# NumericalEarth/Breeze.jl

Measured on AMD Instinct MI355X. Metric: grid-cells advanced/sec (tendency+Poisson step), 512^3 anelastic, higher is better.
Workload: dtype f64

## Files before the change

### breeze.jl_amd/csrc/bz_context.hip

```cpp
#include <cmath>
#include <cstdlib>
#include <cstring>

#include "bz_internal.h"

ProfileScope::ProfileScope(bz_ctx *c, const char *name) : ctx(c)
{
    if (!ctx->profiling || ctx->profile_mute) return;
    for (size_t s = 0; s < ctx->slots.size(); ++s)
        if (ctx->slots[s].name == name || std::strcmp(ctx->slots[s].name, name) == 0) slot = (int)s;
    if (slot < 0) {
        ctx->slots.emplace_back();
        ctx->slots.back().name = name;
        slot = (int)ctx->slots.size() - 1;
    }
    if (hipEventCreate(&e0) != hipSuccess || hipEventCreate(&e1) != hipSuccess) { slot = -1; return; }
    hipEventRecord(e0, ctx->stream);
}
ProfileScope::~ProfileScope()
{
    if (slot < 0) return;
    hipEventRecord(e1, ctx->stream);
    ctx->slots[slot].pending.emplace_back(e0, e1);
}
// ... 13 lines not shown
        }
        s.pending.clear();
    }
}

void bzi_read_tuning(bz_tuning &t)
{
    auto on = [](const char *n) { return getenv(n) != nullptr; };
    auto num = [](const char *n, int d) { const char *e = getenv(n); return e ? atoi(e) : d; };
    t.no_fused = on("BZ_NO_FUSED");
    t.no_fuse_rk = on("BZ_NO_FUSE_RK");
    t.no_lean = on("BZ_NO_LEAN");
    t.no_xcd = on("BZ_NO_XCD");
    t.no_k6_stored = on("BZ_NO_K6_STORED");
    t.no_closure_march = on("BZ_NO_CLOSURE_MARCH");
    t.no_dry_shortcut = on("BZ_NO_DRY_SHORTCUT");
    t.side_scalar = on("BZ_SIDE_SCALAR");
    t.no_fuse_forcing = on("BZ_NO_FUSE_FORCING");
    t.no_fold_forcing = on("BZ_NO_FOLD_FORCING");
    t.no_fuse_level_sums = on("BZ_NO_FUSE_LEVEL_SUMS");
    t.ac_xcd = num("BZ_AC_XCD", 1);
    t.ac_forward2 = num("BZ_AC_FWD2", 1);
    t.ac_pfold = num("BZ_AC_PFOLD", 1);
    t.ac_init_fold = num("BZ_AC_INIT_FOLD", 1);
    t.ac_pair_avg = num("BZ_AC_PAIR_AVG", 1);
    t.ac_rotate = num("BZ_AC_ROTATE", 1);
    t.ac_cfg = num("BZ_AC_CFG", 29);
    t.ac_bx = num("BZ_AC_BX", 128);
    t.no_tridiag_coop = on("BZ_NO_TRIDIAG_COOP");
    t.no_xfft = on("BZ_NO_XFFT");
    t.poisson_kxmajor = num("BZ_POISSON_KXMAJOR", 1);
    t.poisson_kx_pad = num("BZ_POISSON_KX_PAD", 1);
    t.poisson_kx_chunk_kb = num("BZ_POISSON_KX_CHUNK_KB", 0);
    t.poisson_chunk = num("BZ_POISSON_CHUNK", 0);
    t.no_generic_march = on("BZ_NO_GENERIC_MARCH");
    t.no_rho3d_exchange = on("BZ_NO_RHO3D_EXCHANGE");
    t.scalar_lds = num("BZ_SCALAR_LDS", 1);
    t.no_ac_fuse = on("BZ_NO_AC_FUSE");
    t.no_ac_end_fuse = on("BZ_NO_AC_END_FUSE");
    t.comm_no_overlap = on("BZ_COMM_NO_OVERLAP");
    t.comm_self_messages = on("BZ_COMM_SELF_MESSAGES");
    t.comm_no_side_scalar = on("BZ_COMM_NO_SIDE_SCALAR");
    t.nmc_store_always = on("BZ_NMC_STORE_ALWAYS");
    t.graph = num("BZ_GRAPH", -1);
    t.graph_debug = on("BZ_GRAPH_DEBUG");
}

extern "C" int bz_profile_enable(bz_ctx *ctx, int on)
{
    if (!ctx) return BZ_ERR_INVALID;
    if (!on) profile_drain(ctx);
    ctx->profiling = on != 0;
    return BZ_OK;
}
extern "C" int bz_profile_reset(bz_ctx *ctx)
{
    if (!ctx) return BZ_ERR_INVALID;
    profile_drain(ctx);
    for (auto &s : ctx->slots) { s.total_ms = 0.0; s.launches = 0; }
    return BZ_OK;
}
extern "C" int bz_profile_count(bz_ctx *ctx) { return ctx ? (int)ctx->slots.size() : 0; }
extern "C" int bz_profile_get(bz_ctx *ctx, int idx, const char **name, double *total_ms, int64_t *launches)
{
    if (!ctx || idx < 0 || idx >= (int)ctx->slots.size()) return BZ_ERR_INVALID;
    profile_drain(ctx);
// ... 331 lines not shown
```

### breeze.jl_amd/csrc/bz_fused.hip

```cpp
#include "bz_internal.h"

#define FX 64
#define FY 4

struct RKFieldsW {
    double *u[5];
    double *u0[5];
    const double *G[5];
};

template <bool FIRST>
__global__ __launch_bounds__(256) void k_rk3_rows(DevGrid g, RKFieldsW F, double dt, double alpha)
{
    const long long t = (long long)blockIdx.x * 256 + threadIdx.x;
    if (t >= (long long)g.Ny * g.Sx) return;
    const int k = blockIdx.y;
    const long long n = g.Sxy * (k + g.Hz) + (long long)g.Hy * g.Sx + t;
    const double oma = 1.0 - alpha;
#pragma unroll
    for (int f = 0; f < 5; ++f) {
        if (f == 2 && k == 0) continue;
        double u = F.u[f][n];
        if (FIRST) {
            F.u0[f][n] = u;
// ... 320 lines not shown
        if (!once[1]) { BZ_HIP(hipFuncSetAttribute((const void *)k_x_forward<0, 2>, hipFuncAttributeMaxDynamicSharedMemorySize, (int)lds)); once[1] = true; }
        if (rows) hipLaunchKernelGGL((k_x_forward<0, 2>), grid, block, lds, ctx->stream, g, rows, pu, pv, pw, dt, out, L, W, kc);
        else hipLaunchKernelGGL((k_x_forward<1, 2>), grid, block, lds, ctx->stream, g, rows, pu, pv, pw, dt, out, L, W, kc);
    } else if (rows) hipLaunchKernelGGL((k_x_forward<0, 1>), grid, block, lds, ctx->stream, g, rows, pu, pv, pw, dt, out, L, W, kc);
    else hipLaunchKernelGGL((k_x_forward<1, 1>), grid, block, lds, ctx->stream, g, rows, pu, pv, pw, dt, out, L, W, kc);
    BZ_LAUNCH_CHECK();
    return BZ_OK;
}

int bzi_xf_inverse(bz_ctx *ctx, const double *hat, double *phi, int blocks, int klo, int khi)
{
    const DevGrid &g = ctx->dg;
    if (khi <= 0) { klo = 0; khi = g.Nz; }
    const int n2 = g.Nx / 2, kc = xf_chunk(16, g);
    XfLayout L;
    L.nkx = blocks > 1 ? ctx->nkx : n2 + 1;
    L.nxp = blocks > 1 ? ctx->nkx * blocks : n2 + 1;
    L.blk = (long long)g.Nz * L.nkx * g.Ny;
    L.klo = klo; L.khi = khi;
    L.kxs = (ctx->kxmajor && blocks == 1 && !hat) ? (long long)(g.Nz + ctx->kx_pad) * g.Ny : 0;
    const double2 *in = (const double2 *)(hat ? hat : (const double *)ctx->d_hat);
    double *out = phi ? phi : ctx->d_rhs;
    const dim3 grid(g.Ny / XF_RB, (khi - klo + kc - 1) / kc), block(XF_RB * (n2 / 4));
    const size_t lds = xf_lds_bytes(n2);
    if (n2 / 4 > 64 || n2 % 3 == 0) {
        static bool once = false;
        if (!once) { BZ_HIP(hipFuncSetAttribute((const void *)k_x_inverse<2>, hipFuncAttributeMaxDynamicSharedMemorySize, (int)lds)); once = true; }
        hipLaunchKernelGGL(k_x_inverse<2>, grid, block, lds, ctx->stream, g, in, L, out, (const double2 *)ctx->d_wtab, kc);
    } else hipLaunchKernelGGL(k_x_inverse<1>, grid, block, lds, ctx->stream, g, in, L, out, (const double2 *)ctx->d_wtab, kc);
    BZ_LAUNCH_CHECK();
    return BZ_OK;
}

int bzi_rk3_fused(bz_ctx *ctx, const bz_state *s, const bz_prognostic *U0, const bz_prognostic *G, double dt,
                  double alpha, bool first)
{
    const DevGrid &g = ctx->dg;
    ProfileScope ps(ctx, first ? "ssp_rk3_substep+store_initial_state" : "ssp_rk3_substep");
    RKFieldsW F;
    F.u[0] = s->rho_u; F.u[1] = s->rho_v; F.u[2] = s->rho_w; F.u[3] = s->rho_theta; F.u[4] = s->rho_q;
    F.u0[0] = U0->rho_u; F.u0[1] = U0->rho_v; F.u0[2] = U0->rho_w; F.u0[3] = U0->rho_theta; F.u0[4] = U0->rho_q;
    F.G[0] = G->rho_u; F.G[1] = G->rho_v; F.G[2] = G->rho_w; F.G[3] = G->rho_theta; F.G[4] = G->rho_q;
    long long per_level = (long long)g.Ny * g.Sx;
    dim3 grid((unsigned)((per_level + 255) / 256), g.Nz), block(256);
    if (first)
        hipLaunchKernelGGL(k_rk3_rows<true>, grid, block, 0, ctx->stream, g, F, dt, alpha);
    else
        hipLaunchKernelGGL(k_rk3_rows<false>, grid, block, 0, ctx->stream, g, F, dt, alpha);
    BZ_LAUNCH_CHECK();
    return BZ_OK;
}

int bzi_poisson_source_fused(bz_ctx *ctx, const bz_state *s, double dt, double *rhs, const bz_prognostic *predictor)
{
    const DevGrid &g = ctx->dg;
    ProfileScope ps(ctx, "poisson_source_term");
    const int k0 = ctx->krn ? ctx->kr0 : 0, nk = ctx->krn ? ctx->krn : g.Nz;
    dim3 grid((g.Nx + 255) / 256, g.Ny, nk), block(256);
    hipLaunchKernelGGL(k_poisson_source_rows, grid, block, 0, ctx->stream, g, rhs ? rhs : ctx->d_rhs,
                       predictor ? predictor->rho_u : s->rho_u, predictor ? predictor->rho_v : s->rho_v,
                       predictor ? predictor->rho_w : s->rho_w, dt, k0);
    BZ_LAUNCH_CHECK();
    return BZ_OK;
}

int bzi_project_lean(bz_ctx *ctx, const bz_state *s, double dt, const double *phi_c, const double *phi_below,
// ... 58 lines not shown
```

### breeze.jl_amd/csrc/bz_internal.h

```cpp
#pragma once
#include <hip/hip_runtime.h>
#include <hipfft/hipfft.h>

#include <cstdint>
#include <cstdio>
#include <string>
#include <vector>

#include "../../include/breeze_hip.h"

struct ColPtr {
    const double *p = nullptr;
    ColPtr() = default;
    __host__ __device__ ColPtr(const double *q) : p(q) {}
    __host__ __device__ operator const double *() const { return p; }
#ifdef __HIPCC__
    typedef const double __attribute__((address_space(4))) *cptr;
    __device__ __forceinline__ double operator[](int k) const { return ((cptr)p)[k]; }
    __device__ __forceinline__ double operator[](long long k) const { return ((cptr)p)[k]; }
#endif
};

struct DevGrid {
    int Nx, Ny, Nz;
// ... 327 lines not shown

struct BzComm;
struct ProfileSlot {
    const char *name;
    double total_ms = 0.0;
    int64_t launches = 0;
    std::vector<std::pair<hipEvent_t, hipEvent_t>> pending;
};

struct bz_tuning {
    bool no_fused = false;
    bool no_fuse_rk = false;
    bool no_lean = false;
    bool no_xcd = false;
    bool no_closure_march = false;
    bool no_k6_stored = false;
    bool no_dry_shortcut = false;
    bool side_scalar = false;
    bool no_fuse_forcing = false;
    bool no_fold_forcing = false;
    int ac_xcd = 1;
    int ac_forward2 = 1;
    int ac_rotate = 1;
    int ac_pair_avg = 1;
    int ac_init_fold = 1;
    int ac_pfold = 1;
    int ac_bx = 128;
    int ac_cfg = 29;
    bool no_fuse_level_sums = false;
    bool no_tridiag_coop = false;
    bool no_xfft = false;
    int poisson_kxmajor = 1;
    int poisson_kx_chunk_kb = 0;
    int poisson_kx_pad = 1;
    int poisson_chunk = 0;
    int scalar_lds = 1;
    bool no_rho3d_exchange = false;
    bool no_generic_march = false;
    bool no_ac_fuse = false;
    bool no_ac_end_fuse = false;
    bool comm_no_overlap = false;
    bool comm_self_messages = false;
    bool comm_no_side_scalar = false;
    bool nmc_store_always = false;
    int graph = -1;
    bool graph_debug = false;
};
void bzi_read_tuning(bz_tuning &t);
#define BZ_REJECT_BOUNDED_Y(ctx, enabling, what)                                                                             \
    do {                                                                                                                     \
        if ((ctx) && (ctx)->dg.bounded_y && (enabling)) {                                                                                \
            (ctx)->last_error = what ": not implemented on a Bounded y (topology (Periodic, Bounded, Bounded))";            \
            return BZ_ERR_UNSUPPORTED;                                                                                       \
        }                                                                                                                    \
    } while (0)
#define BZ_REJECT_KINEMATIC(ctx, who)                                                                                        \
    do {                                                                                                                     \
        if ((ctx) && (ctx)->kinematic) {                                                                                     \
            (ctx)->last_error = who ": the context has PrescribedDynamics (no momentum, no pressure solve); use bz_time_steps_kinematic"; \
            return BZ_ERR_UNSUPPORTED;                                                                                       \
        }                                                                                                                    \
    } while (0)
#define BZ_HALO_XFACE 8
#define BZ_HALO_YFACE 4
struct bz_ctx;
bool bzi_lean_forcings_ok(const bz_ctx *ctx);

struct bz_ctx {
    bz_tuning tune;
    bz_grid grid;
    bz_constants constants;
    DevGrid dg;
    hipStream_t stream = nullptr;
    bool walls_lean_ok = false;
    int num_cus = 256;
    std::string last_error;

    double *d_columns = nullptr;
    int NXH = 0;
    hipfftHandle plan_fwd = 0, plan_inv = 0;
    hipfftDoubleComplex *d_dctx = nullptr;
    bool plans_ok = false;
    hipfftHandle plan_fwd_c = 0, plan_inv_c = 0;
    int pchunk = 0;
    int kr0 = 0, krn = 0;
    bool xf = false;
    bool xf_slab = false;
    void *d_wtab = nullptr;
    hipfftHandle plan_y = 0;
    bool kxmajor = false;
    int kx_cw = 0, kx_nch = 0, kx_pad = 0;
    hipfftHandle plan_yc = 0, plan_yc_last = 0;
    int profile_mute = 0;
    hipfftHandle slab_plan_x_fwd = 0, slab_plan_x_inv = 0, slab_plan_y = 0;
    bool slab_plans_ok = false;
    int slab_inv_ld = 0;
    double *d_rhs = nullptr;
    hipfftDoubleComplex *d_hat = nullptr;
    double *d_ibeta = nullptr;
    double *d_tfac = nullptr;
    double *d_lower = nullptr;
    double *d_scalar = nullptr;
    double *d_havg = nullptr;
    double *d_moments = nullptr;
    struct AzPlan *az = nullptr;
    int y_nranks = 1, y_rank = 0, nkx = 0, kx0 = 0, Ny_global = 0;
    bool slab_mode = false;
    bool tiled_tendencies = true;
    bool fuse_rk = true;
    bool G_is_predictor = false;
    bool fused_ok = true;
    int q_host = 0;
    int *h_qstate = nullptr;
    hipEvent_t ev_q = nullptr;
    bool q_pending = false;
    int *d_qstate = nullptr;
    bool diagnostics_stale = false;
    bool lean_step_last = false;
    bool lean = true;
    bool lean_xcd = true;
    hipStream_t side_stream = nullptr;
// ... 190 lines not shown
                       int32_t unpack, int sx, long long sxy);
int bzi_comm_join_pending(bz_ctx *ctx);
int bzi_refresh_diagnostics(bz_ctx *ctx, const bz_state *s, const char *who);
int bzi_kinematic_update_state(bz_ctx *ctx, const bz_state *s, const bz_prognostic *G, int compute_tendencies);
void bzi_kinematic_teardown(bz_ctx *ctx);
enum bz_tier { BZ_TIER_LEAN, BZ_TIER_FUSED_RK, BZ_TIER_FUSED, BZ_TIER_OPERATORS };
bz_tier bzi_anelastic_tier(const bz_ctx *ctx);
inline constexpr double BZ_SSP_RK3_ALPHA[3] = {1.0, 1.0 / 4.0, 2.0 / 3.0};
int bzi_zero_wall_faces(bz_ctx *ctx, const bz_prognostic *G, const bz_prognostic *U0 = nullptr);
int bzi_fused_rk_physics(bz_ctx *ctx, const bz_state *s, const bz_prognostic *G, double dt, double alpha, bool first, bool fold);
void bzi_lean_step_done(bz_ctx *ctx, bool diagnosed);
int bzi_scan_moisture(bz_ctx *ctx, const bz_state *s);
int bzi_scan_moisture_field(bz_ctx *ctx, const double *rho_q);
const int *bzi_moisture_state(const bz_ctx *ctx);
void bzi_moisture_unknown(bz_ctx *ctx);
struct LeanStage;
void bzi_lean_stage(const bz_state *s, const bz_prognostic *U0, const bz_prognostic *G, int stage, LeanStage *L);
int bzi_dist_time_step_compressible(bz_ctx *ctx, const bz_compressible_state *s, const bz_compressible_prognostic *U0,
                                    const bz_compressible_prognostic *G, const bz_acoustic_substepper *sub, double dt);
int bzi_compressible_store_initial_state(bz_ctx *ctx, const bz_compressible_state *s, const bz_compressible_prognostic *U0);
void bzi_comm_teardown(bz_ctx *ctx);
int bzi_comm_allreduce_sum(bz_ctx *ctx, double *buf, int n);
void bzi_lean_teardown(bz_ctx *ctx);
void bzi_poisson_teardown(bz_ctx *ctx);
int bzi_poisson_solve(bz_ctx *ctx, const bz_state *s, double dt);
int bzi_poisson_spectral(bz_ctx *ctx);
int bzi_poisson_from_momentum(bz_ctx *ctx, const bz_state *s, double dt, const bz_prognostic *predictor);
int bzi_fft_chunk(bz_ctx *ctx, int k0, bool forward);
int bzi_xf_forward(bz_ctx *ctx, const bz_state *s, double dt, const bz_prognostic *predictor, const double *rhs = nullptr,
                   double *hat = nullptr, int blocks = 1, int klo = 0, int khi = 0);
int bzi_xf_inverse(bz_ctx *ctx, const double *hat = nullptr, double *phi = nullptr, int blocks = 1, int klo = 0, int khi = 0);
int bzi_xf_y(bz_ctx *ctx, bool forward);
int bzi_tridiag_launch(bz_ctx *ctx, double *hat, double scale, int Ny, int mean_column, int kx_lo = 0, int kx_hi = 0);
int bzi_xf_middle(bz_ctx *ctx);
int bzi_rk3_fused(bz_ctx *ctx, const bz_state *s, const bz_prognostic *U0, const bz_prognostic *G, double dt,
                  double alpha, bool first);
int bzi_poisson_source_fused(bz_ctx *ctx, const bz_state *s, double dt, double *rhs = nullptr,
                             const bz_prognostic *predictor = nullptr);
int bzi_project_diagnose(bz_ctx *ctx, const bz_state *s, double dt, const double *phi_c = nullptr,
                         const double *phi_below = nullptr, const bz_prognostic *predictor = nullptr, bool store_phi = true,
                         const double *rtheta_in = nullptr, const double *rq_in = nullptr, bool level_sums = false);
int bzi_project_lean(bz_ctx *ctx, const bz_state *s, double dt, const double *phi_c, const double *phi_below,
                     const bz_prognostic *predictor, double *sa, double *sb);
struct LeanStage {
    bz_state sin;
    bz_state sout;
    bz_prognostic u0;
    const double *pa, *pb;
    double *oa, *ob;
};
int bzi_tendencies_lean(bz_ctx *ctx, const bz_state *s, const bz_prognostic *U0, const bz_prognostic *G, const double *pa,
                        const double *pb, double *oa, double *ob, double dt, double alpha, bool first, int rows = 0, int which = 3);
static inline int bzi_lean_tendencies(bz_ctx *ctx, const LeanStage &L, const bz_prognostic *G, double dt, double alpha, bool first,
                                      int rows = 0, int which = 3)
{
    return bzi_tendencies_lean(ctx, &L.sin, &L.u0, G, L.pa, L.pb, L.oa, L.ob, dt, alpha, first, rows, which);
}
int bzi_scalar_pair_fork(bz_ctx *ctx, const LeanStage &L, const bz_prognostic *G, double dt, double alpha, bool first);
int bzi_scalar_pair_join(bz_ctx *ctx);
int bzi_tendencies_fused_rk(bz_ctx *ctx, const bz_state *s, const bz_prognostic *U0, const bz_prognostic *G, double dt,
                            double alpha, bool first);
int bzi_create(bz_ctx **out, const bz_grid *grid, const bz_constants *constants, const bz_reference_state *ref,
               int weno_order, int y_nranks, int y_rank, bool slab_mode, bool compressible = false);
void bzi_compressible_teardown(bz_ctx *ctx);
int bzi_cmp_surface_fluxes(bz_ctx *ctx, const bz_compressible_state *s, const bz_compressible_prognostic *G);
void bzi_cmp_surface_flux_teardown(bz_ctx *ctx);
// ... 13 lines not shown
```

### breeze.jl_amd/csrc/bz_poisson.hip

```cpp
#include <cmath>
#include <cstdlib>

#include "bz_internal.h"
#include "bz_weno.h"

#define TX 64
#define TY 4

__global__ __launch_bounds__(TX *TY) void k_poisson_source(DevGrid g, double *__restrict__ rhs,
                                                          const double *__restrict__ ru,
                                                          const double *__restrict__ rv,
                                                          const double *__restrict__ rw, double dt)
{
    int i = blockIdx.x * TX + threadIdx.x, j = blockIdx.y * TY + threadIdx.y, k = blockIdx.z;
    if (i >= g.Nx || j >= g.Ny) return;
    long long n = g.idx(i, j, k);
    double Ax = g.Ax[k], Ay = g.Ay[k], Az = g.Az;
    double a = Ax * ru[n + 1] - Ax * ru[n];
    double b = g.flat_y ? 0.0 : Ay * rv[n + g.Sx] - Ay * rv[n];
    double c = Az * rw[n + g.Sxy] - Az * rw[n];
    double div = g.Vinv_c[k] * (a + b + c);
    rhs[(long long)i + (long long)g.Nx * ((long long)j + (long long)g.Ny * k)] = g.dzc[k] * div / dt;
}

// ... 383 lines not shown
    double *d_diag0 = d_cols + Nz, *d_mass = d_cols + 2 * Nz, *d_lx = d_cols + 3 * Nz, *d_ly = d_lx + nxh_real;
    BZ_HIP(hipMemcpy(ctx->d_lower, lower.data(), Nz * sizeof(double), hipMemcpyHostToDevice));
    BZ_HIP(hipMemcpy(d_diag0, diag0.data(), Nz * sizeof(double), hipMemcpyHostToDevice));
    BZ_HIP(hipMemcpy(d_mass, mass.data(), Nz * sizeof(double), hipMemcpyHostToDevice));
    BZ_HIP(hipMemcpy(d_lx, lam_x.data(), nxh_real * sizeof(double), hipMemcpyHostToDevice));
    BZ_HIP(hipMemcpy(d_ly, lam_y.data(), Ny * sizeof(double), hipMemcpyHostToDevice));

    if (!slab) {
        BZ_HIP(hipMalloc(&ctx->d_rhs, nreal * sizeof(double)));
        BZ_HIP(hipMalloc(&ctx->d_hat, (nhat + (size_t)ctx->NXH * 4 * Ny) * sizeof(hipfftDoubleComplex)));
        BZ_HIP(hipMemset(ctx->d_hat, 0, (nhat + (size_t)ctx->NXH * 4 * Ny) * sizeof(hipfftDoubleComplex)));
    }
    BZ_HIP(hipMalloc(&ctx->d_ibeta, nhat * sizeof(double)));
    BZ_HIP(hipMalloc(&ctx->d_tfac, nhat * sizeof(double)));

    TriCols C{ctx->d_lower, d_diag0, d_mass, d_lx, d_ly};
    long long plane = (long long)ctx->NXH * Ny;
    hipLaunchKernelGGL(k_tridiag_setup, dim3((unsigned)((plane + 255) / 256)), dim3(256), 0, 0, ctx->NXH, Ny, Nz, ctx->kx0, nxh_real, (slab || ctx->xf) ? 1 : 0, C,
                       ctx->d_ibeta, ctx->d_tfac);
    BZ_HIP(hipGetLastError());
    BZ_HIP(hipDeviceSynchronize());

    if (ctx->xf || ctx->xf_slab) {
        const int nw = 3 * Nx / 4;
        std::vector<double> w(2 * (size_t)nw);
        for (int t = 0; t < nw; ++t) {
            const double a = (double)(2.0 * pi * (double)t / (double)Nx);
            w[2 * t] = std::cos(a);
            w[2 * t + 1] = -std::sin(a);
        }
        BZ_HIP(hipMalloc(&ctx->d_wtab, w.size() * sizeof(double)));
        BZ_HIP(hipMemcpy(ctx->d_wtab, w.data(), w.size() * sizeof(double), hipMemcpyHostToDevice));
    }
    if (slab) return BZ_OK;
    int n[2] = {Ny, Nx};
    if (g.bounded_x)
        BZ_HIP(hipMalloc(&ctx->d_dctx, (size_t)(Nx / 2 + 1) * Nz * sizeof(hipfftDoubleComplex)));
    if (!ctx->xf && Ny == 1) {
        int n1[1] = {Nx};
        BZ_FFT(hipfftPlanMany(&ctx->plan_fwd, 1, n1, nullptr, 1, 0, nullptr, 1, 0, HIPFFT_D2Z, Nz));
        BZ_FFT(hipfftPlanMany(&ctx->plan_inv, 1, n1, nullptr, 1, 0, nullptr, 1, 0, HIPFFT_Z2D, Nz));
        ctx->plans_ok = true;
        BZ_FFT(hipfftSetStream(ctx->plan_fwd, ctx->stream));
        BZ_FFT(hipfftSetStream(ctx->plan_inv, ctx->stream));
    } else if (!ctx->xf) {
        BZ_FFT(hipfftPlanMany(&ctx->plan_fwd, 2, n, nullptr, 1, 0, nullptr, 1, 0, HIPFFT_D2Z, Nz));
        BZ_FFT(hipfftPlanMany(&ctx->plan_inv, 2, n, nullptr, 1, 0, nullptr, 1, 0, HIPFFT_Z2D, Nz));
        ctx->plans_ok = true;
        BZ_FFT(hipfftSetStream(ctx->plan_fwd, ctx->stream));
        BZ_FFT(hipfftSetStream(ctx->plan_inv, ctx->stream));
    }
    if (ctx->xf) {
        int ny[1] = {Ny};
        BZ_FFT(hipfftPlanMany(&ctx->plan_y, 1, ny, ny, 1, Ny, ny, 1, Ny, HIPFFT_Z2Z, ctx->NXH * Nz));
        BZ_FFT(hipfftSetStream(ctx->plan_y, ctx->stream));
        const size_t spec = (size_t)ctx->NXH * Nz * Ny * sizeof(hipfftDoubleComplex);
        constexpr size_t KX_CHUNK_MB = 256;
        const size_t chunk_bytes = ctx->tune.poisson_kx_chunk_kb > 0 ? (size_t)ctx->tune.poisson_kx_chunk_kb << 10
                                   : KX_CHUNK_MB << 20;
        if (ctx->tune.poisson_kxmajor && !g.bounded_y && tridiag_coop_segs(ctx, Ny) && Ny % TCO_COLS == 0 && spec > chunk_bytes + chunk_bytes / 2) {
            const int nch = (int)((spec + chunk_bytes - 1) / chunk_bytes);
            ctx->kx_cw = (ctx->NXH + nch - 1) / nch;
            ctx->kx_nch = (ctx->NXH + ctx->kx_cw - 1) / ctx->kx_cw;
            const int last = ctx->NXH - (ctx->kx_nch - 1) * ctx->kx_cw;
            ctx->kx_pad = std::max(0, std::min(4, ctx->tune.poisson_kx_pad));
            const int lines = Nz + ctx->kx_pad;
            BZ_FFT(hipfftPlanMany(&ctx->plan_yc, 1, ny, ny, 1, Ny, ny, 1, Ny, HIPFFT_Z2Z, ctx->kx_cw * lines));
            BZ_FFT(hipfftSetStream(ctx->plan_yc, ctx->stream));
            if (last != ctx->kx_cw) {
                BZ_FFT(hipfftPlanMany(&ctx->plan_yc_last, 1, ny, ny, 1, Ny, ny, 1, Ny, HIPFFT_Z2Z, last * lines));
                BZ_FFT(hipfftSetStream(ctx->plan_yc_last, ctx->stream));
            }
            ctx->kxmajor = true;
        }
    }
    int ch = ctx->tune.poisson_chunk;
    if (ch > 0 && ch < Nz && Nz % ch == 0 && !ctx->xf) {
        BZ_FFT(hipfftPlanMany(&ctx->plan_fwd_c, 2, n, nullptr, 1, 0, nullptr, 1, 0, HIPFFT_D2Z, ch));
        BZ_FFT(hipfftPlanMany(&ctx->plan_inv_c, 2, n, nullptr, 1, 0, nullptr, 1, 0, HIPFFT_Z2D, ch));
        BZ_FFT(hipfftSetStream(ctx->plan_fwd_c, ctx->stream));
        BZ_FFT(hipfftSetStream(ctx->plan_inv_c, ctx->stream));
        ctx->pchunk = ch;
    }
    return BZ_OK;
}

int bzi_fft_chunk(bz_ctx *ctx, int k0, bool forward)
{
    const DevGrid &g = ctx->dg;
    double *real = ctx->d_rhs + (size_t)g.Nx * g.Ny * k0;
    hipfftDoubleComplex *hat = ctx->d_hat + (size_t)ctx->NXH * g.Ny * k0;
    if (forward) BZ_FFT(hipfftExecD2Z(ctx->plan_fwd_c, real, hat));
    else BZ_FFT(hipfftExecZ2D(ctx->plan_inv_c, hat, real));
    return BZ_OK;
}

void bzi_poisson_teardown(bz_ctx *ctx)
{
    if (ctx->slab_plans_ok) {
        hipfftDestroy(ctx->slab_plan_x_fwd);
        hipfftDestroy(ctx->slab_plan_x_inv);
        hipfftDestroy(ctx->slab_plan_y);
        ctx->slab_plans_ok = false;
    }
    if (ctx->xf && ctx->plan_y) hipfftDestroy(ctx->plan_y);
    if (ctx->plan_yc) hipfftDestroy(ctx->plan_yc);
    if (ctx->plan_yc_last) hipfftDestroy(ctx->plan_yc_last);
    ctx->plan_yc = ctx->plan_yc_last = 0; ctx->kxmajor = false;
    if (ctx->d_wtab) hipFree(ctx->d_wtab);
    ctx->plan_y = 0; ctx->d_wtab = nullptr; ctx->xf = ctx->xf_slab = false;
    if (ctx->plans_ok) {
        hipfftDestroy(ctx->plan_fwd);
        hipfftDestroy(ctx->plan_inv);
        if (ctx->pchunk) { hipfftDestroy(ctx->plan_fwd_c); hipfftDestroy(ctx->plan_inv_c); ctx->pchunk = 0; }
        ctx->plans_ok = false;
    }
    if (ctx->d_dctx) hipFree(ctx->d_dctx);
    ctx->d_dctx = nullptr;
    if (ctx->d_lower) hipFree(ctx->d_lower);
    if (ctx->d_rhs) hipFree(ctx->d_rhs);
    if (ctx->d_hat) hipFree(ctx->d_hat);
    if (ctx->d_ibeta) hipFree(ctx->d_ibeta);
    if (ctx->d_tfac) hipFree(ctx->d_tfac);
    ctx->d_lower = ctx->d_rhs = ctx->d_ibeta = ctx->d_tfac = nullptr;
    ctx->d_hat = nullptr;
}

template <int MODE>
__global__ __launch_bounds__(256) void k_dct_line(double2 *__restrict__ hat, int N)
{
    extern __shared__ double2 dct_line[];
    double2 *line = hat + (long long)blockIdx.x * N;
    for (int m = threadIdx.x; m < N; m += 256) dct_line[m] = line[m];
    __syncthreads();
    for (int m = threadIdx.x; m < N; m += 256) {
        double2 out;
        if (MODE == 0) out = (m < N / 2) ? dct_line[2 * m] : dct_line[2 * (N - 1 - m) + 1];
        else if (MODE == 3) out = (m & 1) ? dct_line[N - 1 - (m - 1) / 2] : dct_line[m / 2];
        else {
            const double ang = 3.14159265358979323846 * (double)m / (2.0 * (double)N);
            const double sn = sin(ang), cs = cos(ang);
            if (MODE == 1) {
// ... 13 lines not shown
__global__ __launch_bounds__(256) void k_dctx_row(double *__restrict__ real, double2 *__restrict__ half, double2 *__restrict__ full, int N)
{
    extern __shared__ double2 dct_line[];
    const int NH = N / 2 + 1;
    const long long row = blockIdx.x;
    if (MODE == 0 || MODE == 3) {
        double *sm = (double *)dct_line, *x = real + row * N;
        for (int m = threadIdx.x; m < N; m += 256) sm[m] = x[m];
        __syncthreads();
        for (int m = threadIdx.x; m < N; m += 256)
            x[m] = (MODE == 0) ? ((m < N / 2) ? sm[2 * m] : sm[2 * (N - 1 - m) + 1]) : ((m & 1) ? sm[N - 1 - (m - 1) / 2] : sm[m / 2]);
    } else if (MODE == 1) {
        const double2 *V = half + row * NH;
        for (int m = threadIdx.x; m < N; m += 256) {
            const double ang = 3.14159265358979323846 * (double)m / (2.0 * (double)N);
            const double sn = sin(ang), cs = cos(ang);
            const double2 v = (m <= N / 2) ? V[m] : make_double2(V[N - m].x, -V[N - m].y);
            full[row * N + m] = make_double2(2.0 * (cs * v.x + sn * v.y), 0.0);
        }
    } else {
        const double2 *X = full + row * N;
        for (int m = threadIdx.x; m < NH; m += 256) {
            const double ang = 3.14159265358979323846 * (double)m / (2.0 * (double)N);
            const double sn = sin(ang), cs = cos(ang);
            const double a = X[m].x, b = m ? X[N - m].x : 0.0;
            half[row * NH + m] = make_double2(0.5 * (cs * a + sn * b), 0.5 * (sn * a - cs * b));
        }
    }
}

int bzi_xf_y(bz_ctx *ctx, bool forward)
{
    const DevGrid &g = ctx->dg;
    if (!g.bounded_y) {
        BZ_FFT(hipfftExecZ2Z(ctx->plan_y, ctx->d_hat, ctx->d_hat, forward ? HIPFFT_FORWARD : HIPFFT_BACKWARD));
        return BZ_OK;
    }
    const unsigned lines = (unsigned)(ctx->NXH * g.Nz);
    const size_t lds = (size_t)g.Ny * sizeof(double2);
    double2 *hat = (double2 *)ctx->d_hat;
    if (forward) {
        hipLaunchKernelGGL(k_dct_line<0>, dim3(lines), dim3(256), lds, ctx->stream, hat, g.Ny);
        BZ_FFT(hipfftExecZ2Z(ctx->plan_y, ctx->d_hat, ctx->d_hat, HIPFFT_FORWARD));
        hipLaunchKernelGGL(k_dct_line<1>, dim3(lines), dim3(256), lds, ctx->stream, hat, g.Ny);
    } else {
        hipLaunchKernelGGL(k_dct_line<2>, dim3(lines), dim3(256), lds, ctx->stream, hat, g.Ny);
        BZ_FFT(hipfftExecZ2Z(ctx->plan_y, ctx->d_hat, ctx->d_hat, HIPFFT_BACKWARD));
        hipLaunchKernelGGL(k_dct_line<3>, dim3(lines), dim3(256), lds, ctx->stream, hat, g.Ny);
    }
    BZ_LAUNCH_CHECK();
    return BZ_OK;
}

int bzi_xf_middle(bz_ctx *ctx)
{
    const DevGrid &g = ctx->dg;
    const double scale = 1.0 / ((double)g.Nx * (double)g.Ny);
    int rc;
    if (ctx->kxmajor) {
        ProfileScope ps(ctx, "poisson_fft_y+tridiagonal");
        hipfftDoubleComplex *hat = (hipfftDoubleComplex *)ctx->d_hat;
        for (int c = 0; c < ctx->kx_nch; ++c) {
            const int kx_lo = c * ctx->kx_cw, kx_hi = std::min(ctx->NXH, kx_lo + ctx->kx_cw);
            hipfftHandle plan = (kx_hi - kx_lo == ctx->kx_cw) ? ctx->plan_yc : ctx->plan_yc_last;
            hipfftDoubleComplex *p = hat + (size_t)kx_lo * (g.Nz + ctx->kx_pad) * g.Ny;
            BZ_FFT(hipfftExecZ2Z(plan, p, p, HIPFFT_FORWARD));
            if ((rc = bzi_tridiag_launch(ctx, (double *)ctx->d_hat, scale, g.Ny, 1, kx_lo, kx_hi))) return rc;
            BZ_FFT(hipfftExecZ2Z(plan, p, p, HIPFFT_BACKWARD));
        }
        return BZ_OK;
    }
    {
        ProfileScope ps(ctx, "poisson_fft_y_forward");
        if ((rc = bzi_xf_y(ctx, true))) return rc;
    }
    {
        ProfileScope ps(ctx, "poisson_tridiagonal");
        if ((rc = bzi_tridiag_launch(ctx, (double *)ctx->d_hat, scale, g.Ny, 1))) return rc;
    }
    ProfileScope ps(ctx, "poisson_fft_y_inverse");
    return bzi_xf_y(ctx, false);
}

int bzi_poisson_spectral(bz_ctx *ctx)
{
    const DevGrid &g = ctx->dg;
    if (ctx->xf) {
        int rc;
        {
            ProfileScope ps(ctx, "poisson_fft_x_forward");
            if ((rc = bzi_xf_forward(ctx, nullptr, 1.0, nullptr))) return rc;
        }
        if ((rc = bzi_xf_middle(ctx))) return rc;
        ProfileScope ps(ctx, "poisson_fft_x_inverse");
        return bzi_xf_inverse(ctx);
    }
    const size_t lds_x = (size_t)g.Nx * sizeof(double);
    {
        ProfileScope ps(ctx, "poisson_fft_forward");
        if (g.bounded_x) {
            hipLaunchKernelGGL(k_dctx_row<0>, dim3(g.Nz), dim3(256), lds_x, ctx->stream, ctx->d_rhs, nullptr, nullptr, g.Nx);
// ... 76 lines not shown
```

### breeze.jl_amd/csrc/bz_xfft_kernels.h

```cpp
#pragma once

typedef double xf_pair2 __attribute__((ext_vector_type(2), aligned(sizeof(double))));
#define XF_RB 8

__device__ __forceinline__ void xf_block(int &bj, int &bk)
{
    bj = blockIdx.x; bk = blockIdx.y;
    const unsigned gx = gridDim.x;
    if ((gx & 7u) == 0) {
        const unsigned w = blockIdx.y * gx + blockIdx.x, c = w & 7u, r = w >> 3, band = gx >> 3;
        bj = (int)(c * band + r % band);
        bk = (int)(r / band);
    }
}

__device__ __forceinline__ int xf_slot(int p, int n2)
{
    const int h = p >> 4;
    const int x = ((h & 2) ? 6 : 0) ^ ((h & 4) ? 15 : 0) ^ ((h & 8) ? 9 : 0);
    return (p < n2) ? (p ^ x) : p;
}
#define XF_P(p) xf_slot((p), n2)
#define XF_ROW_STRIDE(n2) ((n2) + 4)

// ... 125 lines not shown
            row[XF_P(n2)] = make_double2(z.x - z.y, 0.0);
        } else {
            const int m = n2 - p;
            const double2 A = row[XF_P(p)], B = row[XF_P(m)];
            const double2 E = make_double2(0.5 * (A.x + B.x), 0.5 * (A.y - B.y));
            const double2 D = make_double2(0.5 * (A.x - B.x), 0.5 * (A.y + B.y));
            const double2 WD = xf_cmul(W[p], D);
            row[XF_P(p)] = make_double2(E.x + WD.y, E.y - WD.x);
            row[XF_P(m)] = make_double2(E.x - WD.y, -(E.y + WD.x));
        }
    }
}
__device__ __forceinline__ void xf_split_inverse(double2 *__restrict__ row, int n2, int tid, const double2 *__restrict__ W)
{
    const int T = n2 >> 2;
    for (int p = tid; p <= (n2 >> 1); p += T) {
        if (p == 0) {
            const double a = row[0].x, b = row[XF_P(n2)].x;
            row[0] = make_double2(a + b, a - b);
        } else {
            const int m = n2 - p;
            const double2 P = row[XF_P(p)], Q = row[XF_P(m)];
            const double2 S = make_double2(P.x + Q.x, P.y - Q.y);
            const double2 Dd = make_double2(P.x - Q.x, P.y + Q.y);
            double2 w = W[p];
            w.y = -w.y;
            const double2 V = xf_cmul(w, Dd);
            row[XF_P(p)] = make_double2(S.x - V.y, S.y + V.x);
            row[XF_P(m)] = make_double2(S.x + V.y, -(S.y - V.x));
        }
    }
}

struct XfLayout {
    int nkx, nxp;
    long long blk;
    int klo, khi;
    long long kxs;
};
__device__ __forceinline__ long long xf_addr(const XfLayout &L, int Ny, int k, int kx, int row)
{
    if (L.kxs) return (long long)kx * L.kxs + (long long)k * Ny + row;
    const int d = kx / L.nkx, kxl = kx - d * L.nkx;
    return (long long)d * L.blk + ((long long)k * L.nkx + kxl) * Ny + row;
}

template <int SRC, int TW = 1>
__global__ __launch_bounds__(XF_RB * 64 * TW) void k_x_forward(DevGrid g, const double *__restrict__ rhs, const double *__restrict__ ru,
                                                          const double *__restrict__ rv, const double *__restrict__ rw, double dt,
                                                          double2 *__restrict__ hatT, XfLayout L, const double2 *__restrict__ Wg, int kchunk)
{
    extern __shared__ double2 xf_sm[];
    const int Nx = g.Nx, n2 = Nx >> 1, T = n2 >> 2, RS = XF_ROW_STRIDE(n2), NXH = n2 + 1;
    const int nthreads = blockDim.x;
    const int r = threadIdx.x / T, tid = threadIdx.x - r * T;
    double2 *__restrict__ W = xf_sm + XF_RB * RS;
    const int wn = xf_w_entries(n2);
    double2 *__restrict__ Wst = W + wn;
    for (int t = threadIdx.x; t < wn; t += nthreads) W[t] = Wg[t];
    xf_stage_twiddles(Wst, Wg, n2, threadIdx.x, nthreads);
    __syncthreads();
    int bj, bk;
    xf_block(bj, bk);
    const int j0 = bj * XF_RB, j = j0 + r;
    const int kbeg = L.klo + bk * kchunk, kend = min(kbeg + kchunk, L.khi);
    double2 *__restrict__ row = xf_sm + r * RS;
// ... 54 lines not shown
    const int Nx = g.Nx, n2 = Nx >> 1, T = n2 >> 2, RS = XF_ROW_STRIDE(n2), NXH = n2 + 1;
    const int nthreads = blockDim.x;
    const int r = threadIdx.x / T, tid = threadIdx.x - r * T;
    double2 *__restrict__ W = xf_sm + XF_RB * RS;
    const int wn = xf_w_entries(n2);
    double2 *__restrict__ Wst = W + wn;
    for (int t = threadIdx.x; t < wn; t += nthreads) W[t] = Wg[t];
    xf_stage_twiddles(Wst, Wg, n2, threadIdx.x, nthreads);
    int bj, bk;
    xf_block(bj, bk);
    const int j0 = bj * XF_RB;
    const int kbeg = L.klo + bk * kchunk, kend = min(kbeg + kchunk, L.khi);
    double2 *__restrict__ row = xf_sm + r * RS;
    for (int k = kbeg; k < kend; ++k) {
        for (int e = threadIdx.x; e < NXH * XF_RB; e += nthreads) {
            const int kx = e / XF_RB, rr = e - kx * XF_RB;
            xf_sm[rr * RS + XF_P(kx)] = hatT[xf_addr(L, g.Ny, k, kx, j0 + rr)];
        }
        __syncthreads();
        xf_split_inverse(row, n2, tid, W);
        xf_sync<TW>();
        xf_team_fft<true, TW>(row, n2, tid, true, W, Wst);
        {
            double *dst = phi_c + (long long)Nx * ((long long)(j0 + r) + (long long)g.Ny * k);
#pragma unroll
            for (int q = 0; q < 4; ++q) {
                const int c = tid + T * q;
                *(double2 *)(dst + 2 * c) = row[XF_P(c)];
            }
        }
        __syncthreads();
    }
}
```

Measured before the change: 4.234 billion.

## Replace hipFFT y-direction transforms with custom Stockham radix-8/16 LDS kernel

Adds a hand-written batched complex FFT kernel for power-of-two Ny (8..512). Each row is transformed in registers with radix-8 or radix-16 butterflies, using swizzled LDS for the exchanges and a twiddle table cached in LDS. The kernel replaces the hipFFT Z2Z calls in both the standard and kx-major chunked Poisson paths. The aim is to avoid hipFFT's generic-plan overhead and extra memory passes. It also adds a knob that forces the kx chunk width. The risk is that the custom kernel may be less efficient than the vendor library, or introduce numerical mismatches.

```diff
diff --git a/breeze.jl_amd/csrc/bz_context.hip b/breeze.jl_amd/csrc/bz_context.hip
--- a/breeze.jl_amd/csrc/bz_context.hip
+++ b/breeze.jl_amd/csrc/bz_context.hip
@@ -69,6 +69,8 @@
     t.poisson_kxmajor = num("BZ_POISSON_KXMAJOR", 1);
     t.poisson_kx_pad = num("BZ_POISSON_KX_PAD", 1);
     t.poisson_kx_chunk_kb = num("BZ_POISSON_KX_CHUNK_KB", 0);
+    t.poisson_kx_chunk_wn = num("BZ_POISSON_KX_CHUNK_WAVENUMBERS", 0);
+    t.no_yfft = on("BZ_NO_YFFT");
     t.poisson_chunk = num("BZ_POISSON_CHUNK", 0);
     t.no_generic_march = on("BZ_NO_GENERIC_MARCH");
     t.no_rho3d_exchange = on("BZ_NO_RHO3D_EXCHANGE");
diff --git a/breeze.jl_amd/csrc/bz_fused.hip b/breeze.jl_amd/csrc/bz_fused.hip
--- a/breeze.jl_amd/csrc/bz_fused.hip
+++ b/breeze.jl_amd/csrc/bz_fused.hip
@@ -376,6 +376,25 @@
     return BZ_OK;
 }
 
+bool bzi_yfft_covers(int Ny) { return Ny >= 8 && Ny <= 512 && (Ny & (Ny - 1)) == 0; }
+
+int bzi_yfft(bz_ctx *ctx, double *hat, long long nrows, bool forward)
+{
+    const int n = ctx->dg.Ny;
+    const bool r8 = n == 8 || n == 512;
+    const int R = r8 ? 8 : 16, rpb = 2048 / n;
+    const size_t lds = (size_t)(2048 + n / 2) * sizeof(double2);
+    const dim3 grid((unsigned)((nrows + rpb - 1) / rpb)), block(2048 / R);
+    double2 *p = (double2 *)hat;
+    const double2 *W = (const double2 *)ctx->d_wtab_y;
+    if (r8 && forward) hipLaunchKernelGGL((k_y_fft<8, false>), grid, block, lds, ctx->stream, p, nrows, n, W);
+    else if (r8) hipLaunchKernelGGL((k_y_fft<8, true>), grid, block, lds, ctx->stream, p, nrows, n, W);
+    else if (forward) hipLaunchKernelGGL((k_y_fft<16, false>), grid, block, lds, ctx->stream, p, nrows, n, W);
+    else hipLaunchKernelGGL((k_y_fft<16, true>), grid, block, lds, ctx->stream, p, nrows, n, W);
+    BZ_LAUNCH_CHECK();
+    return BZ_OK;
+}
+
 int bzi_rk3_fused(bz_ctx *ctx, const bz_state *s, const bz_prognostic *U0, const bz_prognostic *G, double dt,
                   double alpha, bool first)
 {
diff --git a/breeze.jl_amd/csrc/bz_internal.h b/breeze.jl_amd/csrc/bz_internal.h
--- a/breeze.jl_amd/csrc/bz_internal.h
+++ b/breeze.jl_amd/csrc/bz_internal.h
@@ -383,6 +383,8 @@
     bool no_xfft = false;
     int poisson_kxmajor = 1;
     int poisson_kx_chunk_kb = 0;
+    int poisson_kx_chunk_wn = 0;
+    bool no_yfft = false;
     int poisson_kx_pad = 1;
     int poisson_chunk = 0;
     int scalar_lds = 1;
@@ -438,6 +440,8 @@
     bool xf = false;
     bool xf_slab = false;
     void *d_wtab = nullptr;
+    void *d_wtab_y = nullptr;
+    bool yfft = false;
     hipfftHandle plan_y = 0;
     bool kxmajor = false;
     int kx_cw = 0, kx_nch = 0, kx_pad = 0;
@@ -694,6 +698,8 @@
 int bzi_xf_inverse(bz_ctx *ctx, const double *hat = nullptr, double *phi = nullptr, int blocks = 1, int klo = 0, int khi = 0);
 int bzi_xf_y(bz_ctx *ctx, bool forward);
 int bzi_tridiag_launch(bz_ctx *ctx, double *hat, double scale, int Ny, int mean_column, int kx_lo = 0, int kx_hi = 0);
+bool bzi_yfft_covers(int Ny);
+int bzi_yfft(bz_ctx *ctx, double *hat, long long nrows, bool forward);
 int bzi_xf_middle(bz_ctx *ctx);
 int bzi_rk3_fused(bz_ctx *ctx, const bz_state *s, const bz_prognostic *U0, const bz_prognostic *G, double dt,
                   double alpha, bool first);
diff --git a/breeze.jl_amd/csrc/bz_poisson.hip b/breeze.jl_amd/csrc/bz_poisson.hip
--- a/breeze.jl_amd/csrc/bz_poisson.hip
+++ b/breeze.jl_amd/csrc/bz_poisson.hip
@@ -439,6 +439,17 @@
         BZ_HIP(hipMalloc(&ctx->d_wtab, w.size() * sizeof(double)));
         BZ_HIP(hipMemcpy(ctx->d_wtab, w.data(), w.size() * sizeof(double), hipMemcpyHostToDevice));
     }
+    ctx->yfft = ctx->xf && !g.bounded_y && bzi_yfft_covers(Ny) && !ctx->tune.no_yfft;
+    if (ctx->yfft) {
+        std::vector<double> w((size_t)Ny);
+        for (int t = 0; t < Ny / 2; ++t) {
+            const double a = (double)(2.0 * pi * (double)t / (double)Ny);
+            w[2 * t] = std::cos(a);
+            w[2 * t + 1] = -std::sin(a);
+        }
+        BZ_HIP(hipMalloc(&ctx->d_wtab_y, w.size() * sizeof(double)));
+        BZ_HIP(hipMemcpy(ctx->d_wtab_y, w.data(), w.size() * sizeof(double), hipMemcpyHostToDevice));
+    }
     if (slab) return BZ_OK;
     int n[2] = {Ny, Nx};
     if (g.bounded_x)
@@ -465,16 +476,20 @@
         constexpr size_t KX_CHUNK_MB = 256;
         const size_t chunk_bytes = ctx->tune.poisson_kx_chunk_kb > 0 ? (size_t)ctx->tune.poisson_kx_chunk_kb << 10
                                    : KX_CHUNK_MB << 20;
-        if (ctx->tune.poisson_kxmajor && !g.bounded_y && tridiag_coop_segs(ctx, Ny) && Ny % TCO_COLS == 0 && spec > chunk_bytes + chunk_bytes / 2) {
+        const int forced_cw = std::min(ctx->tune.poisson_kx_chunk_wn, ctx->NXH);
+        if (ctx->tune.poisson_kxmajor && !g.bounded_y && tridiag_coop_segs(ctx, Ny) && Ny % TCO_COLS == 0 &&
+            (forced_cw > 0 || spec > chunk_bytes + chunk_bytes / 2)) {
             const int nch = (int)((spec + chunk_bytes - 1) / chunk_bytes);
-            ctx->kx_cw = (ctx->NXH + nch - 1) / nch;
+            ctx->kx_cw = forced_cw > 0 ? forced_cw : (ctx->NXH + nch - 1) / nch;
             ctx->kx_nch = (ctx->NXH + ctx->kx_cw - 1) / ctx->kx_cw;
             const int last = ctx->NXH - (ctx->kx_nch - 1) * ctx->kx_cw;
             ctx->kx_pad = std::max(0, std::min(4, ctx->tune.poisson_kx_pad));
             const int lines = Nz + ctx->kx_pad;
-            BZ_FFT(hipfftPlanMany(&ctx->plan_yc, 1, ny, ny, 1, Ny, ny, 1, Ny, HIPFFT_Z2Z, ctx->kx_cw * lines));
-            BZ_FFT(hipfftSetStream(ctx->plan_yc, ctx->stream));
-            if (last != ctx->kx_cw) {
+            if (!ctx->yfft) {
+                BZ_FFT(hipfftPlanMany(&ctx->plan_yc, 1, ny, ny, 1, Ny, ny, 1, Ny, HIPFFT_Z2Z, ctx->kx_cw * lines));
+                BZ_FFT(hipfftSetStream(ctx->plan_yc, ctx->stream));
+            }
+            if (!ctx->yfft && last != ctx->kx_cw) {
                 BZ_FFT(hipfftPlanMany(&ctx->plan_yc_last, 1, ny, ny, 1, Ny, ny, 1, Ny, HIPFFT_Z2Z, last * lines));
                 BZ_FFT(hipfftSetStream(ctx->plan_yc_last, ctx->stream));
             }
@@ -515,6 +530,8 @@
     if (ctx->plan_yc_last) hipfftDestroy(ctx->plan_yc_last);
     ctx->plan_yc = ctx->plan_yc_last = 0; ctx->kxmajor = false;
     if (ctx->d_wtab) hipFree(ctx->d_wtab);
+    if (ctx->d_wtab_y) hipFree(ctx->d_wtab_y);
+    ctx->d_wtab_y = nullptr; ctx->yfft = false;
     ctx->plan_y = 0; ctx->d_wtab = nullptr; ctx->xf = ctx->xf_slab = false;
     if (ctx->plans_ok) {
         hipfftDestroy(ctx->plan_fwd);
@@ -594,6 +611,7 @@
 int bzi_xf_y(bz_ctx *ctx, bool forward)
 {
     const DevGrid &g = ctx->dg;
+    if (ctx->yfft) return bzi_yfft(ctx, (double *)ctx->d_hat, (long long)ctx->NXH * g.Nz, forward);
     if (!g.bounded_y) {
         BZ_FFT(hipfftExecZ2Z(ctx->plan_y, ctx->d_hat, ctx->d_hat, forward ? HIPFFT_FORWARD : HIPFFT_BACKWARD));
         return BZ_OK;
@@ -626,9 +644,12 @@
             const int kx_lo = c * ctx->kx_cw, kx_hi = std::min(ctx->NXH, kx_lo + ctx->kx_cw);
             hipfftHandle plan = (kx_hi - kx_lo == ctx->kx_cw) ? ctx->plan_yc : ctx->plan_yc_last;
             hipfftDoubleComplex *p = hat + (size_t)kx_lo * (g.Nz + ctx->kx_pad) * g.Ny;
-            BZ_FFT(hipfftExecZ2Z(plan, p, p, HIPFFT_FORWARD));
+            const long long nrows = (long long)(kx_hi - kx_lo) * (g.Nz + ctx->kx_pad);
+            if (ctx->yfft) { if ((rc = bzi_yfft(ctx, (double *)p, nrows, true))) return rc; }
+            else BZ_FFT(hipfftExecZ2Z(plan, p, p, HIPFFT_FORWARD));
             if ((rc = bzi_tridiag_launch(ctx, (double *)ctx->d_hat, scale, g.Ny, 1, kx_lo, kx_hi))) return rc;
-            BZ_FFT(hipfftExecZ2Z(plan, p, p, HIPFFT_BACKWARD));
+            if (ctx->yfft) { if ((rc = bzi_yfft(ctx, (double *)p, nrows, false))) return rc; }
+            else BZ_FFT(hipfftExecZ2Z(plan, p, p, HIPFFT_BACKWARD));
         }
         return BZ_OK;
     }
diff --git a/breeze.jl_amd/csrc/bz_xfft_kernels.h b/breeze.jl_amd/csrc/bz_xfft_kernels.h
--- a/breeze.jl_amd/csrc/bz_xfft_kernels.h
+++ b/breeze.jl_amd/csrc/bz_xfft_kernels.h
@@ -181,6 +181,111 @@
     }
 }
 
+__device__ __forceinline__ int xr_slot(int p, int n) { return (p < n) ? (p ^ (((p >> 3) ^ (p >> 6)) & 7)) : p; }
+
+__device__ __forceinline__ double2 xr_add(double2 a, double2 b) { return make_double2(a.x + b.x, a.y + b.y); }
+__device__ __forceinline__ double2 xr_sub(double2 a, double2 b) { return make_double2(a.x - b.x, a.y - b.y); }
+template <bool INV>
+__device__ __forceinline__ double2 xr_mulw(double2 a, double c, double s)
+{
+    return INV ? make_double2(a.x * c - a.y * s, a.y * c + a.x * s) : make_double2(a.x * c + a.y * s, a.y * c - a.x * s);
+}
+template <bool INV>
+__device__ __forceinline__ double2 xr_rot(double2 a) { return INV ? make_double2(-a.y, a.x) : make_double2(a.y, -a.x); }
+
+template <bool INV>
+__device__ __forceinline__ void xr_dft4(double2 &a0, double2 &a1, double2 &a2, double2 &a3)
+{
+    const double2 s0 = xr_add(a0, a2), d0 = xr_sub(a0, a2), s1 = xr_add(a1, a3), d1 = xr_rot<INV>(xr_sub(a1, a3));
+    a0 = xr_add(s0, s1); a1 = xr_add(d0, d1); a2 = xr_sub(s0, s1); a3 = xr_sub(d0, d1);
+}
+template <bool INV>
+__device__ __forceinline__ void xr_dft(double2 (&v)[2])
+{
+    const double2 a = v[0], b = v[1];
+    v[0] = xr_add(a, b); v[1] = xr_sub(a, b);
+}
+template <bool INV>
+__device__ __forceinline__ void xr_dft(double2 (&v)[4]) { xr_dft4<INV>(v[0], v[1], v[2], v[3]); }
+template <bool INV>
+__device__ __forceinline__ void xr_dft(double2 (&v)[8])
+{
+    const double H = 0.7071067811865476;
+    xr_dft4<INV>(v[0], v[2], v[4], v[6]);
+    xr_dft4<INV>(v[1], v[3], v[5], v[7]);
+    v[3] = xr_mulw<INV>(v[3], H, H);
+    v[5] = xr_rot<INV>(v[5]);
+    v[7] = xr_mulw<INV>(v[7], -H, H);
+    double2 o[8];
+#pragma unroll
+    for (int q = 0; q < 4; ++q) { o[q] = xr_add(v[2 * q], v[2 * q + 1]); o[q + 4] = xr_sub(v[2 * q], v[2 * q + 1]); }
+#pragma unroll
+    for (int q = 0; q < 8; ++q) v[q] = o[q];
+}
+template <bool INV>
+__device__ __forceinline__ void xr_dft(double2 (&v)[16])
+{
+    const double H = 0.7071067811865476, C1 = 0.9238795325112867, S1 = 0.3826834323650898;
+#pragma unroll
+    for (int p = 0; p < 4; ++p) xr_dft4<INV>(v[p], v[p + 4], v[p + 8], v[p + 12]);
+    v[5] = xr_mulw<INV>(v[5], C1, S1);   v[6] = xr_mulw<INV>(v[6], H, H);     v[7] = xr_mulw<INV>(v[7], S1, C1);
+    v[9] = xr_mulw<INV>(v[9], H, H);     v[10] = xr_rot<INV>(v[10]);          v[11] = xr_mulw<INV>(v[11], -H, H);
+    v[13] = xr_mulw<INV>(v[13], S1, C1); v[14] = xr_mulw<INV>(v[14], -H, H);  v[15] = xr_mulw<INV>(v[15], -C1, -S1);
+#pragma unroll
+    for (int q = 0; q < 4; ++q) xr_dft4<INV>(v[4 * q], v[4 * q + 1], v[4 * q + 2], v[4 * q + 3]);
+    double2 o[16];
+#pragma unroll
+    for (int q = 0; q < 16; ++q) o[(q >> 2) + 4 * (q & 3)] = v[q];
+#pragma unroll
+    for (int q = 0; q < 16; ++q) v[q] = o[q];
+}
+
+template <int R, int r, bool INV>
+__device__ __forceinline__ void xr_butterflies(double2 (&v)[R], int tid, int T, int Ns, const double2 *__restrict__ W, int wq)
+{
+    constexpr int M = R / r;
+#pragma unroll
+    for (int m = 0; m < M; ++m) {
+        double2 a[r];
+#pragma unroll
+        for (int q = 0; q < r; ++q) a[q] = v[m + q * M];
+        if (Ns > 1) {
+            const int k = (tid + m * T) & (Ns - 1);
+            double2 w[r];
+            w[1] = W[k * wq];
+            if (INV) w[1].y = -w[1].y;
+#pragma unroll
+            for (int q = 2; q < r; ++q) w[q] = (q & 1) ? xf_cmul(w[q - 1], w[1]) : xf_cmul(w[q / 2], w[q / 2]);
+#pragma unroll
+            for (int q = 1; q < r; ++q) a[q] = xf_cmul(a[q], w[q]);
+        }
+        xr_dft<INV>(a);
+#pragma unroll
+        for (int q = 0; q < r; ++q) v[m + q * M] = a[q];
+    }
+}
+
+template <int R, bool INV>
+__device__ __forceinline__ void xr_fft(double2 (&v)[R], double2 *__restrict__ row, int n, int tid, const double2 *__restrict__ W, int wbase)
+{
+    const int T = n / R;
+    xr_butterflies<R, R, INV>(v, tid, T, 1, W, 0);
+    for (int done = R; done < n;) {
+        const int Ns = done / R, k = tid & (Ns - 1);
+        xf_wave_sync();
+#pragma unroll
+        for (int q = 0; q < R; ++q) row[xr_slot((tid - k) * R + k + q * Ns, n)] = v[q];
+        xf_wave_sync();
+#pragma unroll
+        for (int c = 0; c < R; ++c) v[c] = row[xr_slot(tid + T * c, n)];
+        const int r = n / done;
+        if (r >= R) { xr_butterflies<R, R, INV>(v, tid, T, done, W, wbase / (done * R)); done *= R; continue; }
+        if (r == 2) xr_butterflies<R, 2, INV>(v, tid, T, done, W, wbase / n);
+        else if (r == 4) xr_butterflies<R, 4, INV>(v, tid, T, done, W, wbase / n);
+        else if constexpr (R == 16) xr_butterflies<R, 8, INV>(v, tid, T, done, W, wbase / n);
+        done = n;
+    }
+}
 struct XfLayout {
     int nkx, nxp;
     long long blk;
@@ -301,3 +406,28 @@
         __syncthreads();
     }
 }
+
+template <int R, bool INV>
+__global__ __launch_bounds__(2048 / R) void k_y_fft(double2 *__restrict__ hat, long long nrows, int n, const double2 *__restrict__ Wg)
+{
+    extern __shared__ double2 xf_sm[];
+    constexpr int NT = 2048 / R;
+    const int T = n / R, rpb = NT / T;
+    const int r = threadIdx.x / T, tid = threadIdx.x - r * T;
+    double2 *__restrict__ W = xf_sm + NT * R;
+    for (int t = threadIdx.x; t < n / 2; t += NT) W[t] = Wg[t];
+    __syncthreads();
+    double2 *__restrict__ row = xf_sm + r * n;
+    for (long long r0 = (long long)blockIdx.x * rpb; r0 < nrows; r0 += (long long)gridDim.x * rpb) {
+        const bool mine = r0 + r < nrows;
+        double2 *__restrict__ line = hat + (mine ? r0 + r : nrows - 1) * n;
+        double2 v[R];
+#pragma unroll
+        for (int c = 0; c < R; ++c) v[c] = line[tid + T * c];
+        xr_fft<R, INV>(v, row, n, tid, W, n);
+        if (mine) {
+#pragma unroll
+            for (int c = 0; c < R; ++c) line[tid + T * c] = v[c];
+        }
+    }
+}
```

Result: no change. 4.232 billion (-0.1%).
